# flo-stilz/Audio-Key-Estimation

Hardware: AMD Instinct MI355X
Metric: clips/s (15 s @ 22.05 kHz), HIP CQT + PitchClassNet forward (higher is better)
Workload: dtype f32 accumulation everywhere; pitch / semitone / layer-0 convolutions: f16 activations x f16 weights (per-channel power-of-two scaled) on MFMA, one product; last layer's pitch-class convolutions and heads: 3-term split-bf16 on MFMA (hi*hi + lo*hi + hi*lo); CQT filter bank: 3-term split-bf16 on MFMA

## Files before the change

### audio-key-estimation_amd/csrc/common.h

```cpp
#pragma once

#include <hip/hip_runtime.h>

#include <atomic>
#include <cstdarg>
#include <cstdint>
#include <cstdio>
#include <cstdlib>
#include <string>
#include <vector>

#include "../../include/ake_hip.h"

namespace ake {

void set_error(const char* fmt, ...);

#define AKE_HIP_CHECK(expr)                                                                  \
    do {                                                                                     \
        hipError_t _e = (expr);                                                              \
        if (_e != hipSuccess) {                                                              \
            ake::set_error("%s failed: %s (%s:%d)", #expr, hipGetErrorString(_e), __FILE__, __LINE__); \
            return AKE_ERR_HIP;                                                              \
        }                                                                                    \
// ... 16 lines not shown
bool prof_active();

struct DeviceOnce {
    std::atomic<uint64_t> done{0};
    static int dev() { int d = 0; (void)hipGetDevice(&d); return d & 63; }
    bool need() const { return !((done.load(std::memory_order_acquire) >> dev()) & 1); }
    void mark() { done.fetch_or(1ull << dev(), std::memory_order_release); }
};

template <typename... K>
int set_lds_limit(int bytes, K... kernels) {
    for (const void* f : {reinterpret_cast<const void*>(kernels)...})
        AKE_HIP_CHECK(hipFuncSetAttribute(f, hipFuncAttributeMaxDynamicSharedMemorySize, bytes));
    return AKE_OK;
}

template <typename... K>
int raise_lds_limit(DeviceOnce& once, int bytes, K... kernels) {
    if (!once.need()) return AKE_OK;
    const int rc = set_lds_limit(bytes, kernels...);
    if (!rc) once.mark();
    return rc;
}

template <typename... P, typename... A>
int launch_untimed(const char* name, void (*kernel)(P...), dim3 grid, dim3 block, size_t lds, hipStream_t s, const A&... args) {
    hipLaunchKernelGGL(kernel, grid, block, lds, s, static_cast<P>(args)...);
    const hipError_t e = hipGetLastError();
    if (e == hipSuccess) return AKE_OK;
    set_error("%s: launch failed: %s (grid %u x %u x %u, block %u x %u x %u, %zu B of dynamic LDS)", name, hipGetErrorString(e), grid.x, grid.y,
              grid.z, block.x, block.y, block.z, lds);
    return AKE_ERR_HIP;
}

template <typename... P, typename... A>
int launch(const char* name, void (*kernel)(P...), dim3 grid, dim3 block, size_t lds, hipStream_t s, const A&... args) {
    ProfScope ps(name, s);
    return launch_untimed(name, kernel, grid, block, lds, s, args...);
}

template <typename... P, typename... A>
int launch_flat(const char* name, void (*kernel)(P...), hipStream_t s, long long total, const A&... args) {
    return launch(name, kernel, dim3(static_cast<unsigned>((total + 255) / 256)), dim3(256), 0, s, args...);
}

__device__ __forceinline__ void lds_dma_16(const uint4* src, unsigned int lds_dst) {
    unsigned int keep;
    asm volatile("s_mov_b32 %0, m0\n\ts_mov_b32 m0, %2\n\ts_nop 0\n\tglobal_load_lds_dwordx4 %1, off\n\ts_mov_b32 m0, %0"
                 : "=&s"(keep) : "v"(src), "s"(lds_dst) : "memory");
}

int pcnet_local_window(const ake_pcnet* net);

inline size_t align_up(size_t v, size_t a) { return (v + a - 1) / a * a; }

struct Carver {
    char* base;
    size_t off;
    size_t cap;
    explicit Carver(void* b, size_t c) : base(static_cast<char*>(b)), off(0), cap(c) {}
    template <typename T>
    T* take(size_t n) {
        off = align_up(off, 256);
        T* p = base ? reinterpret_cast<T*>(base + off) : nullptr;
        off += n * sizeof(T);
        return p;
    }
};

}
```

### audio-key-estimation_amd/csrc/pcnet.hip

```cpp
#include <algorithm>
#include <cmath>
#include <cstdlib>
#include <cstring>
#include <map>
#include <string>
#include <vector>

#include "common.h"
#include "pcnet_kernels.h"
#include "pcnet_bwd_kernels.h"

using namespace ake_k;

namespace {

constexpr double kBnEps = 1e-5;
constexpr size_t kLdsBudget = 64 * 1024;
constexpr size_t kBfFragsPerConv = 14 * 2 * 64 + 64;

struct TensorSpec {
    std::string name;
    int64_t shape[4];
    int ndim;
};
// ... 2422 lines not shown
                    const PackedConv& px = train ? n->p2p[i][j].train : n->p2p[i][j].eval;
                    const int bn = train ? n->p2p[i][j].bn : -1;
                    P2pX3Opts ox;
                    ox.lrelu = !train;
                    if ((rc = run_p2p_f16x3(n, rk.x3[j > 0], px.bf_off, sdesc, in_aff, n->blob_dev + px.b_off, B, P, Ti, out.p, d.out_p,
                                            train ? b.stats + 2 * n->bns[bn].ch_off : nullptr, train ? 2 * n->bn_channels : 0, s, "conv_p2p_f16x3_kernel/p2p", ox)))
                        return rc;
                    if (train && (rc = finalize_bn(bn, static_cast<double>(B) * P * Ti, out.aff))) return rc;
                } else if ((rc = conv(n->p2p[i][j], 0, sdesc, in_aff, B, P, Ti, true, out.p, d.out_p, 0, out.aff, "conv_mfma_kernel/p2p")))
                    return rc;
                sdesc = Src{out.p, d.out_p, nullptr, 0, 0};
                in_aff = out.aff;
            }
            if (last_out == P2pOut::SemiFold) {
            } else if (last_out == P2pOut::Semi) {
                if ((rc = run_fold_max("fold_max_kernel", out.p, nullptr, d.out_p, P / 3, B, Ti, cat, ctot, d.prev_pc, s))) return rc;
            } else if (c.stay_sixth && train) {
                if ((rc = run_fold_max("fold_affine_kernel", out.p, out.aff, d.out_p, P, B, Ti, cat, ctot, d.prev_pc, s))) return rc;
                if ((rc = identity(b.aff_cat[i] + 3 * d.prev_pc, d.out_p))) return rc;
            } else if (c.stay_sixth) {
                if ((rc = fold_maps(i, out.p, d.out_p, P, B, Ti, cat, ctot, d.prev_pc))) return rc;
            } else if ((rc = semi(i, out.p, out.aff, B, P, Ti, cat, ctot, d.prev_pc, train ? b.aff_cat[i] + 3 * d.prev_pc : nullptr))) return rc;
            if (last) return AKE_OK;
            Slot psrc{cat, b.cat_slot(train, i).aff};
            int cin = ctot;
            Slot pdst;
            if (c.resblock && train) {
                if ((rc = res_stack_train(n->pc2pc[i], 1, Src{psrc.p, cin, nullptr, 0, 0}, psrc.aff, B, 12, Ti, b.pcst[i], b.aff_pcst[i],
                                          nullptr, 0, "conv_mfma_kernel/pc2pc")))
                    return rc;
                pdst = b.pc_last(i);
            } else if (c.resblock) {
                if ((rc = res_stack(n->pc2pc[i], 1, Src{psrc.p, cin, nullptr, 0, 0}, B, 12, Ti, b.pca[i], b.pcb[i], nullptr, 0, "conv_mfma_kernel/pc2pc"))) return rc;
                pdst = Slot{b.pca[i], nullptr};
            }
            for (int j = 0; j < c.conv_layers && !c.resblock; ++j) {
                pdst = b.pc_out(train, i, j);
                if ((rc = conv(n->pc2pc[i][j], 1, Src{psrc.p, cin, nullptr, 0, 0}, psrc.aff, B, 12, Ti, true, pdst.p, d.out_pc, 0, pdst.aff, "conv_mfma_kernel/pc2pc")))
                    return rc;
                psrc = pdst; cin = d.out_pc;
            }
            const LayerDims& dn = n->dims[i + 1];
            const int ctn = dn.prev_pc + dn.out_p;
            const int Tn = Ti / tp;
            float* catn = b.cat[i + 1] + (i + 1 == L - 1 ? static_cast<size_t>(c0) * ctn * 12 * Tn : 0);
            if ((rc = time_pool(pdst.p, pdst.aff, B, d.out_pc, 12, Ti, catn, ctn, 0))) return rc;
            if (train && (rc = identity(b.aff_cat[i + 1], d.out_pc))) return rc;
            if ((rc = time_pool(out.p, out.aff, B, d.out_p, P, Ti, b.ppool[i], d.out_p, 0))) return rc;
            pc_cur = catn; p_cur = b.ppool[i]; cp = d.out_p;
        }
        return AKE_OK;
    }

    int tail(int B, const int64_t* seq, float* key_out, float* tonic_out, float* genre_out) {
        const auto& c = n->cfg;
        const int L = c.num_layers, tp = c.time_pool_size;
        const int i = L - 1;
        const int Ti = b.Tl[i];
        const LayerDims& d = n->dims[i];
        int rc;
        Slot psrc = L == 1 ? Slot{b.fold0, nullptr} : b.cat_slot(train, i);
        int cin = L == 1 ? 1 : d.prev_pc + d.out_p;
        const int cout_default = L == 1 ? c.n_filters : d.out_pc;
        const int cout = cout_default;
        Slot pdst;
        const bool pc_bf = r.pc == PcStack::Bf16, pc_fused = r.pc == PcStack::Fused;
        const bool head_bf = r.heads != HeadForm::Generic;
        if (pc_fused) {
            if ((rc = run_pc2pc_fused(n, i, psrc.p, cin, B, Ti, b.pcf, head_bf ? b.feat_cl : nullptr, s))) return rc;
        } else if (pc_bf && (rc = run_nchw_to_cl16(psrc.p, cin, B, Ti, reinterpret_cast<unsigned short*>(b.pcb[i]), s))) return rc;
        const char* const pc_label = L == 1 ? "conv_mfma_kernel/pc2pc0" : "conv_mfma_kernel/pc2pc";
        if (c.resblock && train) {
            if ((rc = res_stack_train(n->pc2pc[i], 1, Src{psrc.p, cin, nullptr, 0, 0}, psrc.aff, B, 12, Ti, b.pcst[i], b.aff_pcst[i], nullptr, 0, pc_label)))
                return rc;
            pdst = b.pc_last(i);
        } else if (c.resblock) {
            if ((rc = res_stack(n->pc2pc[i], 1, Src{psrc.p, cin, nullptr, 0, 0}, B, 12, Ti, b.pca[i], b.pcb[i], nullptr, 0, pc_label))) return rc;
            pdst = Slot{b.pca[i], nullptr};
        }
        if (c.denseblock) {
            if ((rc = dense_stack(i, 1, psrc.p, n->final_ch, cin, B, 12, Ti, b.pca[i], pc_label))) return rc;
            pdst = Slot{psrc.p, nullptr};
        }
        for (int j = 0; j < c.conv_layers && !pc_fused && !c.resblock && !c.denseblock; ++j) {
            pdst = b.pc_out(train, i, j);
            if (pc_bf) {
                const bool last_conv = j == c.conv_layers - 1;
                const unsigned short* in = reinterpret_cast<const unsigned short*>(j == 0 ? b.pcb[i] : b.pc_out(false, i, j - 1).p);
                if ((rc = run_pc_bf16(n, n->pc2pc[i][j].eval, in, B, Ti, true, true, last_conv ? pdst.p : nullptr,
                                      last_conv ? nullptr : reinterpret_cast<unsigned short*>(pdst.p), s, "conv_pc_bf16_kernel/pc2pc")))
                    return rc;
                continue;
            }
            if (r.pc_x3_convs >> j & 1) {
                const PackedConv& pt = n->pc2pc[i][j].train;
                unsigned short* planes = reinterpret_cast<unsigned short*>(b.pcb[i]);
                if ((rc = run_nchw_to_cl16_f16x2(psrc.p, cin, B, Ti, psrc.aff, planes, s))) return rc;
                const int bn = n->pc2pc[i][j].bn;
                PcBf16Opts o;
                o.f16x3 = true; o.stats = b.stats + 2 * n->bns[bn].ch_off; o.stats_stride = 2 * n->bn_channels;
                if ((rc = run_pc_bf16(n, pt, planes, B, Ti, true, false, pdst.p, nullptr, s, "conv_pc_f16x3_kernel/pc2pc", o))) return rc;
                if ((rc = finalize_bn(bn, static_cast<double>(B) * 12 * Ti, pdst.aff))) return rc;
            } else if ((rc = conv(n->pc2pc[i][j], 1, Src{psrc.p, cin, nullptr, 0, 0}, psrc.aff, B, 12, Ti, true, pdst.p, cout, 0, pdst.aff, pc_label)))
                return rc;
            psrc = pdst; cin = cout;
        }
        Slot feat = pdst;
        if (pc_fused) feat = Slot{b.pcf, nullptr};
        else if (L > 1) {
            const int cout = c.denseblock ? n->final_ch : cout_default;
            if ((rc = time_pool(pdst.p, pdst.aff, B, cout, 12, Ti, b.pcf, cout, 0))) return rc;
            feat = Slot{b.pcf, nullptr};
        }
        const int Tf = b.Tf;
        const Head* const heads = n->heads;
        int Tm = Tf;
        bool head_planes_ready = false;
        int pooled_heads = 0;
        unsigned short* feat_cl = b.feat_cl;
        if (head_bf && !pc_fused && (rc = run_nchw_to_cl16(feat.p, n->final_ch, B, Tf, feat_cl, s))) return rc;
        const bool head1_bf = r.heads == HeadForm::Head1 || r.heads == HeadForm::Fused, genre_bf = r.genre_bf;
        const int T1 = r.T1, T2 = r.T2, TpB = r.TpB;
        const int nh_bf = genre_bf ? 3 : 2;
        float* const maps[3] = {b.map_k, b.map_t, b.map_g};
        float* const outs[3] = {key_out, tonic_out, genre_out};
        PoolArgs pool;
        pool.seq = reinterpret_cast<const long long*>(seq);
        pool.n_pool_layers = L - 1; pool.tp = tp; pool.shrink = (c.kernel_size - 1) * c.head_layers; pool.max_pool = c.max_pool; pool.clip0 = 0;
        if (r.heads == HeadForm::Fused) {
            const size_t hf_lds = r.hf_lds;
            HeadsFusedArgs ha;
            std::memset(&ha, 0, sizeof(ha));
            ha.xh = feat_cl; ha.xl = feat_cl + static_cast<long long>(B) * 12 * Tf * 16;
            for (int h = 0; h < nh_bf; ++h) {
                const PackedConv& p0 = heads[h].convs[0].eval;
                const PackedConv& p1 = heads[h].convs[1].eval;
                ha.bfragA[h] = n->bf_frags_dev + p0.bf_off; ha.biasA[h] = n->blob_dev + p0.b_off; ha.KHA[h] = p0.kh;
                ha.bfragB[h] = n->bf_frags_dev + p1.bf_off; ha.biasB[h] = n->blob_dev + p1.b_off; ha.KHB[h] = p1.kh;
                ha.dst[h] = maps[h];
                ha.pout[h] = outs[h];
            }
            if (genre_bf) { ha.hs[0] = 2; ha.hs[1] = 0; ha.hs[2] = 1; }
            else { ha.hs[0] = 0; ha.hs[1] = 1; ha.hs[2] = 1; }
            ha.batch = B; ha.T_in = Tf; ha.T1 = T1; ha.T2 = T2; ha.TpA = T1 + 8; ha.TpB = TpB; ha.JB = (T2 + 15) / 16;
            ha.fin_off = static_cast<int>(hf_lds / sizeof(float)) - 12 * T2;
            ha.pool = pool;
            static ake::DeviceOnce hf_attr;
            if ((rc = ake::raise_lds_limit(hf_attr, 150 * 1024, heads_fused_kernel<3>, heads_fused_kernel<4>))) return rc;
            rc = r.heads_mt == 3 ? ake::launch("heads_fused_kernel", heads_fused_kernel<3>, dim3(nh_bf * B), dim3(512), hf_lds, s, ha)
                                 : ake::launch("heads_fused_kernel", heads_fused_kernel<4>, dim3(nh_bf * B), dim3(512), hf_lds, s, ha);
            if (rc) return rc;
            pooled_heads = nh_bf;
            Tm = T2;
        } else if (head1_bf) {
            Head1BfArgs ha;
            std::memset(&ha, 0, sizeof(ha));
            for (int h = 0; h < nh_bf; ++h) {
                const PackedConv& p0 = heads[h].convs[0].eval;
                const PackedConv& p1 = heads[h].convs[1].eval;
                unsigned short* planes = reinterpret_cast<unsigned short*>(b.head_out(false, h, 0, false).p);
                if (h == 0) {
                    PcBf16Opts tonic;
                    tonic.pc2 = &heads[1].convs[0].eval; tonic.planes_out2 = reinterpret_cast<unsigned short*>(b.head_out(false, 1, 0, false).p);
                    if ((rc = run_pc_bf16(n, p0, feat_cl, B, Tf, false, true, nullptr, planes, s, "conv_pc_bf16_kernel/head", tonic))) return rc;
                }
                if (h == 2 && (rc = run_pc_bf16(n, p0, feat_cl, B, Tf, false, true, nullptr, planes, s, "conv_pc_bf16_kernel/genre_head")))
                    return rc;
                ha.xh[h] = planes; ha.xl[h] = planes + static_cast<long long>(B) * 12 * T1 * 32;
                ha.bfrag[h] = n->bf_frags_dev + p1.bf_off; ha.bias[h] = n->blob_dev + p1.b_off; ha.dst[h] = maps[h];
                ha.KH[h] = p1.kh; ha.circular[h] = p1.kh == 12 ? 1 : 0; ha.H_out[h] = ha.circular[h] ? 12 : 12 - p1.kh + 1;
            }
            ha.T_in = T1; ha.T_out = T2; ha.JB = (T2 + 15) / 16; ha.Tp = TpB;
            size_t lds = std::max(static_cast<size_t>(2) * 12 * ha.Tp * 4 * sizeof(uint4), static_cast<size_t>(8) * kHead1MT * 4 * 64 * sizeof(float));
            if (r.heads_pool) {
                ha.fin_off = static_cast<int>(lds / sizeof(float));
                lds += static_cast<size_t>(12) * T2 * sizeof(float);
                for (int h = 0; h < nh_bf; ++h) ha.pout[h] = outs[h];
                ha.pool = pool;
                pooled_heads = nh_bf;
            }
// ... 23 lines not shown
                    }
                    const int bn = cs.bn;
                    PcBf16Opts o;
                    o.f16x3 = true; o.stats = b.stats + 2 * n->bns[bn].ch_off; o.stats_stride = 2 * n->bn_channels;
                    if ((rc = run_pc_bf16(n, pt, b.feat_cl, B, Tcur, false, false, dst.p, nullptr, s,
                                          h == 2 ? "conv_pc_f16x3_kernel/genre_head" : "conv_pc_f16x3_kernel/head", o)))
                        return rc;
                    const int H_out = heads[h].kind == 2 ? 12 - pt.kh + 1 : 12;
                    if ((rc = finalize_bn(bn, static_cast<double>(B) * H_out * (Tcur - pt.kw + 1), dst.aff))) return rc;
                    continue;
                }
                if (train && lastj && j > 0 && pe.cout == 1 && pe.kw == 7 && !n->raw_w_off.empty()) {
                    const size_t lds = (static_cast<size_t>(hc) * 12 * Tcur + static_cast<size_t>(hc) * pe.kh * 7) * sizeof(float);
                    if (lds <= 150 * 1024 && Tcur - 6 >= 1) {
                        static ake::DeviceOnce hl_attr;
                        if ((rc = ake::raise_lds_limit(hl_attr, 150 * 1024, conv_head_last_kernel))) return rc;
                        if ((rc = ake::launch(h == 2 ? "conv_head_last_kernel/genre" : "conv_head_last_kernel", conv_head_last_kernel, dim3(B), dim3(384), lds, s,
                                              src.p, src.aff, n->blob_dev + n->raw_w_off[cs.w], n->blob_dev + n->raw_w_off[cs.b], dst.p, hc, pe.kh,
                                              heads[h].kind == 2 ? 0 : 1, Tcur, Tcur - 6)))
                            return rc;
                        continue;
                    }
                }
                if ((rc = conv(cs, heads[h].kind, Src{src.p, hc, nullptr, 0, 0}, src.aff, B, 12, Tcur, false, dst.p, pe.cout, 0, dst.aff,
                               h == 2 ? "conv_mfma_kernel/genre_head" : "conv_mfma_kernel/head")))
                    return rc;
            }
            Tm = Tf - c.head_layers * (c.kernel_size - 1);
        }
        if (c.local > 0) {
            AKE_REQUIRE(Tm >= c.local, AKE_ERR_INVALID, "pcnet --local: %d map frames are fewer than the pooling window %d", Tm, c.local);
            LocalPoolArgs la;
            std::memset(&la, 0, sizeof(la));
            la.maps[0] = b.map_k; la.maps[1] = b.map_t; la.maps[2] = c.genre ? b.map_g : nullptr;
            la.outs[0] = key_out; la.outs[1] = tonic_out; la.outs[2] = genre_out;
            la.Tm = Tm; la.Tq = Tm - c.local + 1; la.W = c.local; la.batch = B;
            return ake::launch("local_pool_kernel", local_pool_kernel, dim3(static_cast<unsigned>((static_cast<long long>(B) * 12 * Tm + 255) / 256), 3), dim3(256),
                               0, s, la);
        }
        PoolHeadArgs pa;
        std::memset(&pa, 0, sizeof(pa));
        pa.maps[0] = b.map_k; pa.maps[1] = b.map_t; pa.maps[2] = c.genre ? b.map_g : nullptr;
        for (int h = 0; h < pooled_heads; ++h) pa.maps[h] = nullptr;
        if (!pa.maps[0] && !pa.maps[1] && !pa.maps[2]) return AKE_OK;
        pa.outs[0] = key_out; pa.outs[1] = tonic_out; pa.outs[2] = genre_out;
        pa.rows[0] = 12; pa.rows[1] = 12; pa.rows[2] = 11;
        pa.Tm = Tm; pa.batch = B; pa.pool = pool;
        return ake::launch("head_pool_kernel", head_pool_kernel, dim3((B * 12 + 63) / 64, 3), dim3(64), 0, s, pa);
    }
};

int forward_impl(const ake_pcnet* n, bool train, const float* mel, int batch, int frames, const int64_t* seq_length, float* key_out,
                 float* tonic_out, float* genre_out, float* bn_stats_out, void* workspace, size_t ws_bytes, ake_stream_t stream,
                 bool mel_frames_major = false) {
    AKE_REQUIRE(n && mel && key_out && tonic_out, AKE_ERR_INVALID, "pcnet forward: null argument");
    AKE_REQUIRE(n->finalized, AKE_ERR_STATE, "pcnet: ake_pcnet_finalize has not been called");
    AKE_REQUIRE(train || !n->eval_frags_stale, AKE_ERR_STATE,
                "pcnet: the last weight load was ake_pcnet_load_for_training_f32 (training fragments only): call ake_pcnet_load_from_device_f32 before inference");
    AKE_REQUIRE(batch > 0 && frames > 0, AKE_ERR_INVALID, "pcnet: bad batch/frames");
    AKE_REQUIRE(!n->cfg.genre || genre_out, AKE_ERR_INVALID, "pcnet: genre head enabled but genre_out is null");
    const int chunk = train ? batch : std::min(batch, n->chunk_clips);
    Buffers b;
    int rc = plan_buffers(n, batch, chunk, frames, workspace, &b, train);
    if (rc) return rc;
    AKE_REQUIRE(workspace && ws_bytes >= b.bytes, AKE_ERR_WORKSPACE, "pcnet: workspace %zu < %zu bytes", ws_bytes, b.bytes);
    hipStream_t s = static_cast<hipStream_t>(stream);
    const Route route = build_route(n, train, batch, chunk, frames, mel, workspace, mel_frames_major);
    AKE_REQUIRE(!mel_frames_major || route.frames_major, AKE_ERR_UNSUPPORTED,
                "pcnet: this configuration does not take the frames-major input (ake_pcnet_accepts_frames_major)");
    if (train) AKE_HIP_CHECK(hipMemsetAsync(b.stats, 0, sizeof(double) * 2 * n->bn_channels * kStatSlots, s));
    Fwd f{n, b, s, train, route};
    if ((rc = f.entry(mel, batch))) return rc;
    for (int c0 = 0; c0 < batch && n->cfg.num_layers > 1; c0 += chunk) {
        const int B = std::min(chunk, batch - c0);
        if ((rc = f.pitch_chunk(mel + static_cast<size_t>(c0) * n->cfg.pitches * frames, c0, B))) return rc;
    }
    if ((rc = f.tail(batch, seq_length, key_out, tonic_out, genre_out))) return rc;
    if (train && bn_stats_out)
        AKE_HIP_CHECK(hipMemcpyAsync(bn_stats_out, b.bstats, sizeof(float) * 3 * n->bn_channels, hipMemcpyDeviceToDevice, s));
    return AKE_OK;
}

}

#include "pcnet_backward.h"

size_t ake_pcnet_grad_floats(const ake_pcnet* n) { return n ? n->grad_floats : 0; }

int64_t ake_pcnet_grad_offset(const ake_pcnet* n, const char* name) {
    if (!n || !name) return -1;
    auto it = n->spec_index.find(name);
    if (it == n->spec_index.end()) return -1;
    return static_cast<int64_t>(n->grad_off[it->second]);
}

int ake_pcnet_backward_f32(const ake_pcnet* n, const float* mel, int batch, int frames, const int64_t* seq_length, const float* key_out,
                           const float* d_key, const float* d_tonic, const float* d_genre, float* grads_out, int accumulate,
                           void* workspace, size_t ws_bytes, ake_stream_t stream) {
    AKE_REQUIRE(n && mel && key_out && d_key && d_tonic && grads_out, AKE_ERR_INVALID, "pcnet backward: null argument");
    AKE_REQUIRE(n->finalized, AKE_ERR_STATE, "pcnet: ake_pcnet_finalize has not been called");
    AKE_REQUIRE(!n->cfg.genre || d_genre, AKE_ERR_INVALID, "pcnet backward: genre head enabled but d_genre is null");
    AKE_REQUIRE(!(n->cfg.p2pc_conv && n->cfg.stay_sixth), AKE_ERR_UNSUPPORTED, "pcnet: training a --p2pc_conv --stay_sixth net is not built");
    Buffers b;
    int rc = plan_buffers(n, batch, batch, frames, workspace, &b, true);
    if (rc) return rc;
    AKE_REQUIRE(workspace && ws_bytes >= b.bytes, AKE_ERR_WORKSPACE, "pcnet backward: workspace %zu < %zu bytes", ws_bytes, b.bytes);
    hipStream_t s = static_cast<hipStream_t>(stream);
    AKE_HIP_CHECK(hipMemsetAsync(b.gslots, 0, sizeof(gfx_t) * n->grad_floats * kGradSlots, s));
    AKE_HIP_CHECK(hipMemsetAsync(b.stats2, 0, sizeof(double) * (static_cast<size_t>(3) * n->bn_channels * kBwdStatSlots + n->bns.size() * (kAmaxSlots / 2)), s));
    Bwd bw{n, b, s, b.gslots, batch};
    rc = bw.run(mel, seq_length, d_key, d_tonic, d_genre, key_out);
    if (rc) return rc;
    return launch_flat("grad_reduce_kernel", grad_reduce_kernel, s, n->grad_floats, b.gslots, grads_out, static_cast<long long>(n->grad_floats), accumulate ? 1 : 0);
}

int ake_pcnet_local_frames(const ake_pcnet* n, int frames, int* pooled_frames, int* map_frames) {
    AKE_REQUIRE(n && n->cfg.local > 0, AKE_ERR_STATE, "pcnet: the net was not created with local > 0");
    int t = frames;
    for (int i = 1; i < n->cfg.num_layers; ++i) t /= n->cfg.time_pool_size;
    t -= (n->cfg.kernel_size - 1) * n->cfg.head_layers;
    if (map_frames) *map_frames = t;
    if (pooled_frames) *pooled_frames = t - n->cfg.local + 1;
    return AKE_OK;
}

int ake_pcnet_forward_local_f32(const ake_pcnet* n, const float* mel, int batch, int frames, float* key_out, float* tonic_out, float* genre_out,
                                void* workspace, size_t ws_bytes, ake_stream_t stream) {
    AKE_REQUIRE(n && n->cfg.local > 0, AKE_ERR_STATE, "pcnet: the net was not created with local > 0");
    return forward_impl(n, false, mel, batch, frames, nullptr, key_out, tonic_out, genre_out, nullptr, workspace, ws_bytes, stream);
}
// ... 133 lines not shown
                ake::set_error("tap: '%s' is held as f16 words for the pitch conv that reads it; ake_debug_keep_taps(1) before the forward writes it as f32", name);
                return AKE_ERR_INVALID;
            }
            return set(b.psix[i], d.prev_pc, 36, Ti);
        }
        if (i >= 1 && nm == m + "cat") return set(b.cat[i], d.prev_pc + d.out_p, 12, Ti);
        if (i == L - 1 && i >= 1 && nm == m + "time_pool_pc") return set(b.pcf, d.out_pc, 12, b.Tf);
    }
    const int Tm = b.Tf - (c.kernel_size - 1) * c.head_layers;
    if (nm == "key_map") return set(b.map_k, 1, 12, Tm);
    if (nm == "tonic_map") return set(b.map_t, 1, 12, Tm);
    if (nm == "genre_map" && c.genre) return set(b.map_g, 1, 11, Tm);
    ake::set_error("tap: '%s' is not a materialised activation", name);
    return AKE_ERR_INVALID;
}

int ake_debug_keep_taps(int on) {
    const int old = g_keep_taps;
    g_keep_taps = on != 0;
    return old;
}

int ake_pcnet_tap_info(const ake_pcnet* n, const char* name, int batch, int frames, int64_t shape[4]) {
    float* p = nullptr;
    return tap_lookup(n, name, batch, frames, nullptr, &p, shape);
}

int ake_pcnet_tap_copy(const ake_pcnet* n, const char* name, int batch, int frames, const void* workspace, float* out_dev,
                       ake_stream_t stream) {
    AKE_REQUIRE(workspace && out_dev, AKE_ERR_INVALID, "tap_copy: null argument");
    float* p = nullptr;
    int64_t shape[4];
    int cl = 0;
    long long clip_stride = 0;
    int rc = tap_lookup(n, name, batch, frames, workspace, &p, shape, &cl, &clip_stride);
    if (rc) return rc;
    if (clip_stride) {
        const size_t row = sizeof(float) * shape[1] * shape[2] * shape[3];
        AKE_HIP_CHECK(hipMemcpy2DAsync(out_dev, row, p, sizeof(float) * clip_stride, row, shape[0], hipMemcpyDeviceToDevice, static_cast<hipStream_t>(stream)));
        return AKE_OK;
    }
    if (cl) {
        const long long total = shape[0] * shape[1] * shape[2] * shape[3];
        const unsigned short* h = reinterpret_cast<const unsigned short*>(p);
        return ake::launch_untimed("cl_to_nchw_kernel", cl_to_nchw_kernel, dim3(static_cast<unsigned>((total + 255) / 256)), dim3(256), 0,
                                   static_cast<hipStream_t>(stream), h, cl == 2 ? nullptr : h + total, out_dev, shape[1], shape[2], shape[3], total);
    }
    AKE_HIP_CHECK(hipMemcpyAsync(out_dev, p, sizeof(float) * shape[0] * shape[1] * shape[2] * shape[3], hipMemcpyDeviceToDevice,
                                 static_cast<hipStream_t>(stream)));
    return AKE_OK;
}

}
```

### audio-key-estimation_amd/csrc/pcnet_kernels.h

```cpp
#pragma once

#include <hip/hip_runtime.h>

#include "common.h"

namespace ake_k {

constexpr int TW = 4;
constexpr float kSlope = 0.01f;

struct ConvArgs {
    const float* src0;
    const float* src1;
    long long src0_clip_stride, src1_clip_stride;
    int c0, c1, h1;
    int H;
    int T_in;
    int T_out;
    int H_out;
    int py;
    int pad_l;
    int time_circ;
    const float* w;
    const float* bias;
// ... 163 lines not shown
    for (int k = threadIdx.x; k < 2 * C; k += blockDim.x)
        if (sh[k] != 0) atomicAdd(reinterpret_cast<unsigned long long*>(stats + static_cast<size_t>(blockIdx.x & (kStatSlots - 1)) * stats_stride + k),
                                  static_cast<unsigned long long>(sh[k]));
}

template <bool TRAIN>
__global__ void up_sixth_kernel(const float* __restrict__ src, long long src_clip_stride, const float* __restrict__ in_aff,
                                const float* __restrict__ w, const float* __restrict__ bias, float* __restrict__ dst,
                                double* __restrict__ stats, int stats_stride, int C, int T, long long total) {
    __shared__ long long sh[TRAIN ? 2 * kBlockStatCh : 1];
    if constexpr (TRAIN) block_stats_begin(sh, C);
    const long long i = static_cast<long long>(blockIdx.x) * blockDim.x + threadIdx.x;
    if (i < total) {
        const int t = static_cast<int>(i % T);
        long long q = i / T;
        const int row = static_cast<int>(q % 36);
        q /= 36;
        const int co = static_cast<int>(q % C);
        const long long clip = q / C;
        const int p = row / 3, j = row - 3 * p;
        const float* s = src + clip * src_clip_stride + static_cast<long long>(p) * T + t;
        float acc = bias[co];
        for (int ci = 0; ci < C; ++ci) {
            const float x = s[static_cast<long long>(ci) * 12 * T];
            acc = fmaf(TRAIN ? affine_act(x, in_aff, ci) : x, w[(ci * C + co) * 3 + j], acc);
        }
        if constexpr (TRAIN) {
            dst[i] = acc;
            block_stats_add(sh, co, acc);
        } else dst[i] = acc > 0.f ? acc : acc * kSlope;
    }
    if constexpr (TRAIN) block_stats_end(sh, C, stats, stats_stride);
}

__global__ void time_pool_kernel(const float* __restrict__ src, const float* __restrict__ aff, float* __restrict__ dst, int C, int H, int T, int tp,
                                 int dst_ctot, int dst_coff, long long total) {
    const long long i = static_cast<long long>(blockIdx.x) * blockDim.x + threadIdx.x;
    if (i >= total) return;
    const int To = T / tp;
    const int t = static_cast<int>(i % To);
    long long q = i / To;
    const int y = static_cast<int>(q % H);
    q /= H;
    const int c = static_cast<int>(q % C);
    const long long clip = q / C;
    const float* s = src + ((clip * C + c) * H + y) * T + static_cast<long long>(t) * tp;
    float m = affine_act(s[0], aff, c);
    for (int j = 1; j < tp; ++j) m = fmaxf(m, affine_act(s[j], aff, c));
    dst[((clip * dst_ctot + dst_coff + c) * H + y) * To + t] = m;
}

struct PoolArgs {
    const long long* seq;
    int n_pool_layers;
    int tp;
    int shrink;
    int max_pool;
    int clip0;
};

struct PoolHeadArgs {
    const float* maps[3];
    float* outs[3];
    int rows[3];
    int Tm;
    int batch;
    PoolArgs pool;
};

__device__ __forceinline__ float pool_row(const PoolArgs& p, const float* m, int clip, int Tm, int head) {
    int L = Tm;
    bool use_max = p.max_pool != 0;
    if (p.seq) {
        long long l = p.seq[clip];
        for (int k = 0; k < p.n_pool_layers; ++k) l = l / p.tp;
        L = static_cast<int>(l) - p.shrink;
        if (L > Tm) L = Tm;
        if (L < 0) L = Tm + L > 0 ? Tm + L : 0;
        use_max = use_max && (p.clip0 + clip == 0);
    }
    float v;
    if (use_max) {
        v = -INFINITY;
        for (int t = 0; t < L; ++t) v = fmaxf(v, m[t]);
    } else {
        float sum = 0.f;
        for (int t = 0; t < L; ++t) sum += m[t];
        v = sum / static_cast<float>(L > 0 ? L : 0);
    }
    if (head == 0) v = 1.f / (1.f + expf(-v));
    return v;
}

__global__ void head_pool_kernel(PoolHeadArgs a) {
    const int i = blockIdx.x * blockDim.x + threadIdx.x;
    const int which = blockIdx.y;
    if (a.maps[which] == nullptr) return;
    const int rows = a.rows[which];
    if (i >= a.batch * rows) return;
    a.outs[which][i] = pool_row(a.pool, a.maps[which] + static_cast<long long>(i) * a.Tm, i / rows, a.Tm, which);
}


__global__ void concat_repeat_kernel(const float* __restrict__ src0, int c0, const float* __restrict__ src1, int c1, int h1, float* __restrict__ dst,
                                     int ctot, int H, int T, long long total, const float* __restrict__ aff1 = nullptr) {
    const long long i = static_cast<long long>(blockIdx.x) * blockDim.x + threadIdx.x;
    if (i >= total) return;
    const int t = static_cast<int>(i % T);
    long long r = i / T;
    const int y = static_cast<int>(r % H); r /= H;
    const int c = static_cast<int>(r % (c0 + c1));
    const long long clip = r / (c0 + c1);
    float v = c < c0 ? src0[((clip * c0 + c) * H + y) * T + t] : src1[((clip * c1 + (c - c0)) * h1 + y % h1) * T + t];
    if (aff1 && c >= c0) { const float x = fmaf(v, aff1[3 * (c - c0)], aff1[3 * (c - c0) + 1]); v = x > 0.f ? x : x * aff1[3 * (c - c0) + 2]; }
    dst[((clip * ctot + c) * H + y) * T + t] = v;
}

__global__ void dense_affine_kernel(const float* __restrict__ params, const int* __restrict__ idx, float* __restrict__ out, int n) {
    const int i = blockIdx.x * blockDim.x + threadIdx.x;
    if (i >= n) return;
    const int* o = idx + 5 * i;
    const double sc = static_cast<double>(params[o[0]]) / sqrt(static_cast<double>(params[o[3]]) + 1e-5);
    out[3 * i] = static_cast<float>(sc);
    out[3 * i + 1] = static_cast<float>(static_cast<double>(params[o[1]]) - static_cast<double>(params[o[2]]) * sc);
    out[3 * i + 2] = __int_as_float(o[4]);
}

// ... 1155 lines not shown
            int y = m0 / a.T_out, t = m0 - y * a.T_out;
#pragma unroll
            for (int i = 0; i < 4; ++i) {
                if (m0 + i < Mtot && co < a.cout) {
                    float v = F16X3 ? fmaf(fmaf(accl[F16X3 ? mt : 0][F16X3 ? nt : 0][i], kP2pLoInv, acc[mt][nt][i]), iscale, bias) : acc[mt][nt][i] + bias;
                    if (F16X3) sstat.add(v);
                    if (a.lrelu) v = v > 0.f ? v : v * kSlope;
                    if (OUT_CL) {
                        const long long idx = ((static_cast<long long>(clip) * H_out + y) * a.T_out + t) * a.cl_stride + co;
                        const unsigned int hb = bf16_bits(v);
                        oh[idx] = static_cast<unsigned short>(hb);
                        ol[idx] = static_cast<unsigned short>(bf16_bits(v - __uint_as_float(hb << 16)));
                    } else {
                        float* const d = a.dst + clip * a.dst_clip_stride + (static_cast<long long>(co) * H_out + y) * a.T_out + t;
                        *d = (F16X3 && a.accumulate) ? *d + v : v;
                    }
                }
                if (++t == a.T_out) { t = 0; ++y; }
            }
        }
        if (F16X3 && a.stats) {
            long long st1, st2;
            sstat.fixed(st1, st2);
            st1 += shfl_xor_ll(st1, 16); st2 += shfl_xor_ll(st2, 16);
            st1 += shfl_xor_ll(st1, 32); st2 += shfl_xor_ll(st2, 32);
            if (q == 0 && co < a.cout) {
                double* st = a.stats + static_cast<size_t>((blockIdx.x + 7 * blockIdx.z + wave) & (kStatSlots - 1)) * a.stats_stride;
                fx_add_int(st + 2 * co, st1);
                fx_add_int(st + 2 * co + 1, st2);
            }
        }
    }
}

struct Pc2pcFusedArgs {
    const float* src;
    long long src_clip_stride;
    int cin, n_conv;
    const uint4* bfrag[4];
    const float* bias[4];
    float* pooled;
    unsigned short* fh;
    unsigned short* fl;
    int T, Tp;
};

__global__ __launch_bounds__(1024) void pc2pc_fused_kernel(Pc2pcFusedArgs a) {
    extern __shared__ __attribute__((aligned(16))) uint4 lds4[];
    const int clip = blockIdx.x;
    const int lane = threadIdx.x & 63;
    const int wave = __builtin_amdgcn_readfirstlane(threadIdx.x >> 6);
    const int r16 = lane & 15, q = lane >> 4;
    const int T = a.T, Tp = a.Tp;
    constexpr int MT = 4;
    const int n16 = 12 * Tp * 2;
    uint4* const map0 = lds4;
    uint4* const map1 = lds4 + 2 * n16;
    uint4* const wring = lds4 + 4 * n16;
    constexpr int kRow = 4 * 2 * 64;
    for (int i = threadIdx.x; i < 4 * n16; i += 1024) lds4[i] = make_uint4(0, 0, 0, 0);
    const int wsrc0 = (((threadIdx.x >> 7) * 4) * 2 + ((threadIdx.x >> 6) & 1)) * 64 + (threadIdx.x & 63);
    auto wsrc = [&](int p, int dq) { return wsrc0 + (16 * dq * 2 + p * 2) * 64; };
    if (threadIdx.x < kRow) wring[threadIdx.x] = a.bfrag[0][wsrc(0, 0)];
    __syncthreads();
    {
        const float* src = a.src + clip * a.src_clip_stride;
        for (int i = threadIdx.x; i < 12 * T * 2; i += 1024) {
            const int half = i & 1, pos = i >> 1;
            const int y = pos / T, t = pos - y * T;
            unsigned int hi[4] = {0, 0, 0, 0}, lo[4] = {0, 0, 0, 0};
#pragma unroll
            for (int k = 0; k < 8; ++k) {
                const int c = half * 8 + k;
                const float v = c < a.cin ? src[(static_cast<long long>(c) * 12 + y) * T + t] : 0.f;
                const unsigned int hb = bf16_bits(v);
                hi[k >> 1] |= hb << (16 * (k & 1));
                lo[k >> 1] |= bf16_bits(v - __uint_as_float(hb << 16)) << (16 * (k & 1));
            }
            const int idx = ((y * Tp + t + 3) << 1) + half;
            map0[idx] = make_uint4(hi[0], hi[1], hi[2], hi[3]);
            map0[n16 + idx] = make_uint4(lo[0], lo[1], lo[2], lo[3]);
        }
    }
    __syncthreads();
    const int n_tt = (T + 15) >> 4;
    const bool active = wave < 3 * n_tt;
    const int tt = wave / 3, y0 = 4 * (wave - 3 * tt);
    const int t0 = 16 * tt;
    const int dxq = q >> 1, half = q & 1;
    const int lane_off = ((t0 + r16 + dxq) << 1) + half;
    const int lane_off3 = ((t0 + r16 + 6) << 1) + half;
    auto frag_off = [&](int s, int p) {
        int row = y0 + s + (p == 3 ? dxq : 0);
        row -= row >= 12 ? 12 : 0;
        return ((row * Tp) << 1) + (p == 3 ? lane_off3 : lane_off + 4 * p);
    };
    const int Tf = T / 2;
    float* const pooled_c = a.pooled + static_cast<long long>(clip) * 16 * 12 * Tf;
    unsigned short* const fh_c = a.fh ? a.fh + static_cast<long long>(clip) * 12 * Tf * 16 : nullptr;
    unsigned short* const fl_c = a.fh ? a.fl + static_cast<long long>(clip) * 12 * Tf * 16 : nullptr;
    for (int j = 0; j < a.n_conv; ++j) {
        const uint4* const pH = (j & 1) ? map1 : map0;
        const uint4* const pL = pH + n16;
        unsigned short* const oH = reinterpret_cast<unsigned short*>((j & 1) ? map0 : map1);
        unsigned short* const oL = oH + n16 * 8;
        const bool last = j == a.n_conv - 1;
        const uint4* const bfrag_j = j == 0 ? a.bfrag[0] : (j == 1 ? a.bfrag[1] : (j == 2 ? a.bfrag[2] : a.bfrag[3]));
        const float* const bias_j = j == 0 ? a.bias[0] : (j == 1 ? a.bias[1] : (j == 2 ? a.bias[2] : a.bias[3]));
        const uint4* const bfrag_n = j == 0 ? a.bfrag[1] : (j == 1 ? a.bfrag[2] : a.bfrag[3]);
        {
            f32x4c acc[MT];
#pragma unroll
            for (int mt = 0; mt < MT; ++mt) acc[mt] = f32x4c{0.f, 0.f, 0.f, 0.f};
            bf16x8c fh[4], fl[4];
            int c = 0;
            auto run_p = [&](auto pair_c, const int p) __attribute__((always_inline)) {
                constexpr bool PAIR = decltype(pair_c)::value;
                if (active) {
#pragma unroll
                    for (int s = 0; s < 4; ++s) {
                        const int off = frag_off(s, PAIR ? 3 : p);
                        fh[s] = __builtin_bit_cast(bf16x8c, pH[off]);
                        fl[s] = __builtin_bit_cast(bf16x8c, pL[off]);
                    }
                }
#pragma unroll 1
                for (int dq = 0; dq < 3; ++dq, ++c) {
                    uint4 wpre = make_uint4(0, 0, 0, 0);
                    const bool fetch = threadIdx.x < kRow && (c + 1 < 12 || j + 1 < a.n_conv);
                    if (fetch) wpre = c + 1 < 12 ? bfrag_j[dq < 2 ? wsrc(p, dq + 1) : wsrc(p + 1, 0)] : bfrag_n[wsrc(0, 0)];
                    const uint4* const wr = wring + (c & 1) * kRow + lane;
                    if (active) {
#pragma unroll
                        for (int i = 0; i < 4; i += PAIR ? 2 : 1) {
                            const bf16x8c bh = __builtin_bit_cast(bf16x8c, wr[(i * 2 + 0) * 64]), bl = __builtin_bit_cast(bf16x8c, wr[(i * 2 + 1) * 64]);
#pragma unroll
                            for (int mt = 0; mt < MT; ++mt) acc[mt] = __builtin_amdgcn_mfma_f32_16x16x32_bf16(fh[(mt + i) & 3], bh, acc[mt], 0, 0, 0);
#pragma unroll
                            for (int mt = 0; mt < MT; ++mt) acc[mt] = __builtin_amdgcn_mfma_f32_16x16x32_bf16(fl[(mt + i) & 3], bh, acc[mt], 0, 0, 0);
#pragma unroll
                            for (int mt = 0; mt < MT; ++mt) acc[mt] = __builtin_amdgcn_mfma_f32_16x16x32_bf16(fh[(mt + i) & 3], bl, acc[mt], 0, 0, 0);
#pragma unroll
                            for (int u = 0; u < (PAIR ? 2 : 1); ++u) {
                                const int s_new = 4 * dq + i + 4 + u;
                                if (s_new < 12 + MT - (PAIR ? 2 : 1)) {
                                    const int off = frag_off(s_new, PAIR ? 3 : p);
                                    fh[i + u] = __builtin_bit_cast(bf16x8c, pH[off]);
                                    fl[i + u] = __builtin_bit_cast(bf16x8c, pL[off]);
                                }
                            }
                        }
                    }
                    if (fetch) wring[((c + 1) & 1) * kRow + threadIdx.x] = wpre;
                    if (c + 1 < 12) __syncthreads();
                }
            };
#pragma unroll 1
            for (int p = 0; p < 3; ++p) run_p(std::false_type{}, p);
            run_p(std::true_type{}, 3);
            if (active) {
            const int co = r16;
            const float bias = bias_j[co];
            const int tq0 = t0 + 4 * q;
            if (tq0 < T) {
#pragma unroll
            for (int mt = 0; mt < MT; ++mt) {
                    const int y = y0 + mt;
                    float v[4];
#pragma unroll
                    for (int i = 0; i < 4; ++i) {
                        const float x = acc[mt][i] + bias;
                        v[i] = x > 0.f ? x : x * kSlope;
                    }
                    if (!last) {
#pragma unroll
                        for (int i = 0; i < 4; ++i) {
                            const int e = ((((y * Tp + tq0 + i + 3) << 1) + (co >> 3)) << 3) + (co & 7);
                            const unsigned int hb = bf16_bits(v[i]);
                            oH[e] = static_cast<unsigned short>(hb);
                            oL[e] = static_cast<unsigned short>(bf16_bits(v[i] - __uint_as_float(hb << 16)));
                        }
                    } else {
#pragma unroll
                        for (int i = 0; i < 4; i += 2) {
                            const float pv = fmaxf(v[i], v[i + 1]);
                            const int tq = (tq0 + i) >> 1;
                            pooled_c[(co * 12 + y) * Tf + tq] = pv;
                            if (a.fh) {
                                const int e = (y * Tf + tq) * 16 + co;
                                const unsigned int hb = bf16_bits(pv);
                                fh_c[e] = static_cast<unsigned short>(hb);
                                fl_c[e] = static_cast<unsigned short>(bf16_bits(pv - __uint_as_float(hb << 16)));
                            }
                        }
                    }
            }
            }
            }
        }
        __syncthreads();
    }
}

struct Head1BfArgs {
    const unsigned short* xh[3];
    const unsigned short* xl[3];
    const uint4* bfrag[3];
    const float* bias[3];
    float* dst[3];
    int KH[3], H_out[3], circular[3];
    int T_in, T_out, Tp, JB;
    float* pout[3];
    PoolArgs pool;
    int fin_off;
};

constexpr int kHead1MT = 4;
constexpr int kHead1JB = 5;
__host__ __device__ constexpr int head1_ksteps(int KH) { return KH == 12 ? 12 * 7 : KH * 22; }
constexpr int kHead1PF = 3;

__device__ __forceinline__ void head1_prefetch(const uint4* __restrict__ bg, int nks, int wave, uint4 (&nbh)[kHead1PF], uint4 (&nbl)[kHead1PF]) {
#pragma unroll
    for (int i = 0; i < kHead1PF; ++i) {
        const int kn = wave + 8 * i < nks ? wave + 8 * i : wave;
        nbh[i] = bg[(2 * kn + 0) * 64]; nbl[i] = bg[(2 * kn + 1) * 64];
    }
}

__device__ __forceinline__ void head1_multiply_store(const uint4* __restrict__ bg, int nks, uint4 (&nbh)[kHead1PF], uint4 (&nbl)[kHead1PF], uint4* lds4,
                                                     int Tp, int HO, int circ, int JB, int T_out, int clip, const float* bias_p, float* dst,
                                                     bool keep, int fin_off) {
    constexpr int PF = kHead1PF;
    const int lane = threadIdx.x & 63;
    const int wave = __builtin_amdgcn_readfirstlane(threadIdx.x >> 6);
    const int r16 = lane & 15, q = lane >> 4;
    const uint4* const pH = lds4;
    const uint4* const pL = lds4 + 12 * Tp * 4;
    float* const red = reinterpret_cast<float*>(lds4);
    if (circ) {
        f32x4c acc[kHead1JB];
#pragma unroll
        for (int mt = 0; mt < kHead1JB; ++mt) acc[mt] = f32x4c{0.f, 0.f, 0.f, 0.f};
        for (int ks = wave; ks < nks; ks += 8) {
            const int r = ks / 7, dx = ks - r * 7;
            const bf16x8c bh = __builtin_bit_cast(bf16x8c, nbh[0]);
            const bf16x8c bl = __builtin_bit_cast(bf16x8c, nbl[0]);
#pragma unroll
            for (int i = 0; i + 1 < PF; ++i) { nbh[i] = nbh[i + 1]; nbl[i] = nbl[i + 1]; }
            {
                const int kn = ks + 8 * PF < nks ? ks + 8 * PF : ks;
                nbh[PF - 1] = bg[(2 * kn + 0) * 64]; nbl[PF - 1] = bg[(2 * kn + 1) * 64];
// ... 1287 lines not shown
```

### audio-key-estimation_amd/csrc/pipeline.hip

```cpp
#include "common.h"

namespace {

__global__ void fill_i64_kernel(long long* dst, long long v, int n) {
    const int i = blockIdx.x * blockDim.x + threadIdx.x;
    if (i < n) dst[i] = v;
}

__global__ void frames_i64_kernel(long long* dst, const long long* __restrict__ n_clip, int hop, long long t_max, int n) {
    const int i = blockIdx.x * blockDim.x + threadIdx.x;
    if (i < n) {
        const long long nc = n_clip[i];
        const long long t = nc < 0 ? 0 : 1 + nc / hop;
        dst[i] = t < t_max ? t : t_max;
    }
}

struct PipeCarve {
    float* mel;
    long long* seq;
    void* cqt_ws;
    size_t cqt_bytes;
    void* net_ws;
    size_t net_bytes;
    size_t total;
};

int carve(const ake_cqt_plan* plan, const ake_pcnet* net, int batch, int64_t n, int n_bins, void* ws, PipeCarve* pc) {
    const int64_t T = ake_cqt_num_frames(plan, n);
    AKE_REQUIRE(T > 0, AKE_ERR_INVALID, "pipeline: bad n_samples");
    ake::Carver c(ws, 0);
    pc->mel = c.take<float>(static_cast<size_t>(batch) * n_bins * T);
    pc->seq = c.take<long long>(batch);
    pc->cqt_bytes = ake_cqt_workspace_bytes(plan, batch, n);
    pc->cqt_ws = c.take<char>(pc->cqt_bytes);
    pc->net_bytes = ake_pcnet_workspace_bytes(net, batch, static_cast<int>(T));
    pc->net_ws = c.take<char>(pc->net_bytes);
    pc->total = ake::align_up(c.off, 256);
    return AKE_OK;
}

}

extern "C" {

size_t ake_pipeline_workspace_bytes(const ake_cqt_plan* plan, const ake_pcnet* net, int batch, int64_t n_samples) {
    if (!plan || !net || batch <= 0 || n_samples <= 0) return 0;
    PipeCarve pc;
    if (carve(plan, net, batch, n_samples, ake_cqt_plan_n_bins(plan), nullptr, &pc) != AKE_OK) return 0;
    return pc.total;
}

static int pipeline_impl(const ake_cqt_plan* plan, const ake_pcnet* net, const float* audio_dev, int batch, int64_t n_samples,
                         int64_t audio_stride, const int64_t* n_clip_dev, int hop, float* key_out_dev, float* tonic_out_dev,
                         float* genre_out_dev, void* workspace, size_t workspace_bytes, ake_stream_t stream, const int16_t* pcm16_dev = nullptr);

int ake_pipeline_forward_f32(const ake_cqt_plan* plan, const ake_pcnet* net, const float* audio_dev, int batch,
                             int64_t n_samples, int64_t audio_stride, float* key_out_dev, float* tonic_out_dev,
                             float* genre_out_dev, void* workspace, size_t workspace_bytes, ake_stream_t stream) {
    return pipeline_impl(plan, net, audio_dev, batch, n_samples, audio_stride, nullptr, 0, key_out_dev, tonic_out_dev, genre_out_dev, workspace,
                         workspace_bytes, stream);
}

int ake_pipeline_forward_ragged_f32(const ake_cqt_plan* plan, const ake_pcnet* net, const float* audio_dev, int batch,
                                    int64_t n_max, int64_t audio_stride, const int64_t* n_samples_dev, float* key_out_dev,
                                    float* tonic_out_dev, float* genre_out_dev, void* workspace, size_t workspace_bytes,
                                    ake_stream_t stream) {
    AKE_REQUIRE(n_samples_dev, AKE_ERR_INVALID, "ake_pipeline_forward_ragged_f32: null n_samples_dev");
    AKE_REQUIRE(plan && n_max > 0, AKE_ERR_INVALID, "ake_pipeline_forward_ragged_f32: bad argument");
    return pipeline_impl(plan, net, audio_dev, batch, n_max, audio_stride, n_samples_dev, ake_cqt_plan_hop(plan), key_out_dev, tonic_out_dev,
                         genre_out_dev, workspace, workspace_bytes, stream);
}

int ake_pipeline_forward_pcm16_f32(const ake_cqt_plan* plan, const ake_pcnet* net, const int16_t* audio_dev, int batch, int64_t n_max,
                                   int64_t audio_stride, const int64_t* n_samples_dev, float* key_out_dev, float* tonic_out_dev,
                                   float* genre_out_dev, void* workspace, size_t workspace_bytes, ake_stream_t stream) {
    AKE_REQUIRE(plan && n_max > 0, AKE_ERR_INVALID, "ake_pipeline_forward_pcm16_f32: bad argument");
    return pipeline_impl(plan, net, nullptr, batch, n_max, audio_stride, n_samples_dev, ake_cqt_plan_hop(plan), key_out_dev, tonic_out_dev,
                         genre_out_dev, workspace, workspace_bytes, stream, audio_dev);
}

static int pipeline_impl(const ake_cqt_plan* plan, const ake_pcnet* net, const float* audio_dev, int batch, int64_t n_samples,
                         int64_t audio_stride, const int64_t* n_clip_dev, int hop, float* key_out_dev, float* tonic_out_dev,
                         float* genre_out_dev, void* workspace, size_t workspace_bytes, ake_stream_t stream, const int16_t* pcm16_dev) {
    AKE_REQUIRE(plan && net && (audio_dev || pcm16_dev), AKE_ERR_INVALID, "ake_pipeline_forward_f32: null argument");
    const int n_bins = ake_cqt_plan_n_bins(plan);
    AKE_REQUIRE(n_bins == ake_pcnet_pitches(net), AKE_ERR_INVALID, "pipeline: CQT has %d bins but the net expects %d pitches",
                n_bins, ake_pcnet_pitches(net));
    PipeCarve pc;
    int rc = carve(plan, net, batch, n_samples, n_bins, workspace, &pc);
    if (rc) return rc;
    AKE_REQUIRE(workspace && workspace_bytes >= pc.total, AKE_ERR_WORKSPACE, "pipeline: workspace %zu < %zu bytes", workspace_bytes, pc.total);
    const int64_t T = ake_cqt_num_frames(plan, n_samples);
    hipStream_t s = static_cast<hipStream_t>(stream);
    const bool fm = !n_clip_dev && ake_cqt_frames_major_supported(plan) && ake_pcnet_accepts_frames_major(net, batch, static_cast<int>(T));
    rc = pcm16_dev  ? ake_cqt_logmag_pcm16_f32(plan, pcm16_dev, batch, n_samples, audio_stride, n_clip_dev, nullptr, pc.mel, T, fm ? 1 : 0, pc.cqt_ws, pc.cqt_bytes, stream)
         : n_clip_dev ? ake_cqt_logmag_ragged_f32(plan, audio_dev, batch, n_samples, audio_stride, n_clip_dev, pc.mel, T, pc.cqt_ws, pc.cqt_bytes, stream)
         : fm       ? ake_cqt_logmag_frames_major_f32(plan, audio_dev, batch, n_samples, audio_stride, pc.mel, pc.cqt_ws, pc.cqt_bytes, stream)
                    : ake_cqt_logmag_f32(plan, audio_dev, batch, n_samples, audio_stride, pc.mel, T, pc.cqt_ws, pc.cqt_bytes, stream);
    if (rc) return rc;
    if (n_clip_dev)
        rc = ake::launch_untimed("frames_i64_kernel", frames_i64_kernel, dim3((batch + 255) / 256), dim3(256), 0, s, pc.seq,
                                 reinterpret_cast<const long long*>(n_clip_dev), hop, T, batch);
    else
        rc = ake::launch_untimed("fill_i64_kernel", fill_i64_kernel, dim3((batch + 255) / 256), dim3(256), 0, s, pc.seq, T, batch);
    if (rc) return rc;
    if (fm)
        return ake_pcnet_forward_frames_major_f32(net, pc.mel, batch, static_cast<int>(T), reinterpret_cast<const int64_t*>(pc.seq), key_out_dev,
                                                  tonic_out_dev, genre_out_dev, pc.net_ws, pc.net_bytes, stream);
    return ake_pcnet_forward_f32(net, pc.mel, batch, static_cast<int>(T), reinterpret_cast<const int64_t*>(pc.seq), key_out_dev,
                                 tonic_out_dev, genre_out_dev, pc.net_ws, pc.net_bytes, stream);
}

}
```

Before: 465,100.

## Pass uniform sequence length as scalar and split last time tile across extra waves

For the uniform-length pipeline path, the fill kernel that wrote a per-clip sequence-length array is dropped, and the frame count is passed as a scalar through PoolArgs into the pooling code. That removes one small kernel launch and a global read per clip. Separately, the fused pc2pc conv kernel now uses idle waves when there are five time tiles: waves 12+ take the last tile with three rows each (MT=3) instead of leaving it to fewer waves, which improves wave utilisation but adds code paths and register pressure.

```diff
diff --git a/audio-key-estimation_amd/csrc/common.h b/audio-key-estimation_amd/csrc/common.h
--- a/audio-key-estimation_amd/csrc/common.h
+++ b/audio-key-estimation_amd/csrc/common.h
@@ -92,6 +92,9 @@
 
 int pcnet_local_window(const ake_pcnet* net);
 
+int pcnet_forward_uniform(const ake_pcnet* net, const float* mel, int batch, int frames, long long seq_all, bool frames_major, float* key_out,
+                          float* tonic_out, float* genre_out, void* workspace, size_t ws_bytes, ake_stream_t stream);
+
 inline size_t align_up(size_t v, size_t a) { return (v + a - 1) / a * a; }
 
 struct Carver {
diff --git a/audio-key-estimation_amd/csrc/pcnet.hip b/audio-key-estimation_amd/csrc/pcnet.hip
--- a/audio-key-estimation_amd/csrc/pcnet.hip
+++ b/audio-key-estimation_amd/csrc/pcnet.hip
@@ -2498,7 +2498,7 @@
         return AKE_OK;
     }
 
-    int tail(int B, const int64_t* seq, float* key_out, float* tonic_out, float* genre_out) {
+    int tail(int B, const int64_t* seq, long long seq_all, float* key_out, float* tonic_out, float* genre_out) {
         const auto& c = n->cfg;
         const int L = c.num_layers, tp = c.time_pool_size;
         const int i = L - 1;
@@ -2571,7 +2571,7 @@
         float* const maps[3] = {b.map_k, b.map_t, b.map_g};
         float* const outs[3] = {key_out, tonic_out, genre_out};
         PoolArgs pool;
-        pool.seq = reinterpret_cast<const long long*>(seq);
+        pool.seq = reinterpret_cast<const long long*>(seq); pool.seq_all = seq ? -1 : seq_all;
         pool.n_pool_layers = L - 1; pool.tp = tp; pool.shrink = (c.kernel_size - 1) * c.head_layers; pool.max_pool = c.max_pool; pool.clip0 = 0;
         if (r.heads == HeadForm::Fused) {
             const size_t hf_lds = r.hf_lds;
@@ -2701,7 +2701,7 @@
 
 int forward_impl(const ake_pcnet* n, bool train, const float* mel, int batch, int frames, const int64_t* seq_length, float* key_out,
                  float* tonic_out, float* genre_out, float* bn_stats_out, void* workspace, size_t ws_bytes, ake_stream_t stream,
-                 bool mel_frames_major = false) {
+                 bool mel_frames_major = false, long long seq_all = -1) {
     AKE_REQUIRE(n && mel && key_out && tonic_out, AKE_ERR_INVALID, "pcnet forward: null argument");
     AKE_REQUIRE(n->finalized, AKE_ERR_STATE, "pcnet: ake_pcnet_finalize has not been called");
     AKE_REQUIRE(train || !n->eval_frags_stale, AKE_ERR_STATE,
@@ -2724,7 +2724,7 @@
         const int B = std::min(chunk, batch - c0);
         if ((rc = f.pitch_chunk(mel + static_cast<size_t>(c0) * n->cfg.pitches * frames, c0, B))) return rc;
     }
-    if ((rc = f.tail(batch, seq_length, key_out, tonic_out, genre_out))) return rc;
+    if ((rc = f.tail(batch, seq_length, seq_all, key_out, tonic_out, genre_out))) return rc;
     if (train && bn_stats_out)
         AKE_HIP_CHECK(hipMemcpyAsync(bn_stats_out, b.bstats, sizeof(float) * 3 * n->bn_channels, hipMemcpyDeviceToDevice, s));
     return AKE_OK;
@@ -2964,3 +2964,11 @@
 }
 
 }
+
+int ake::pcnet_forward_uniform(const ake_pcnet* n, const float* mel, int batch, int frames, long long seq_all, bool frames_major, float* key_out,
+                               float* tonic_out, float* genre_out, void* workspace, size_t ws_bytes, ake_stream_t stream) {
+    AKE_REQUIRE(!n || n->cfg.local == 0 || frames_major, AKE_ERR_STATE, "pcnet: a --local net returns per-frame outputs: call ake_pcnet_forward_local_f32");
+    AKE_REQUIRE(!n || n->cfg.local == 0, AKE_ERR_UNSUPPORTED, "pcnet: a --local net does not take the frames-major input");
+    AKE_REQUIRE(seq_all >= 0, AKE_ERR_INVALID, "pcnet: bad uniform seq_length %lld", seq_all);
+    return forward_impl(n, false, mel, batch, frames, nullptr, key_out, tonic_out, genre_out, nullptr, workspace, ws_bytes, stream, frames_major, seq_all);
+}
diff --git a/audio-key-estimation_amd/csrc/pcnet_kernels.h b/audio-key-estimation_amd/csrc/pcnet_kernels.h
--- a/audio-key-estimation_amd/csrc/pcnet_kernels.h
+++ b/audio-key-estimation_amd/csrc/pcnet_kernels.h
@@ -239,6 +239,7 @@
 
 struct PoolArgs {
     const long long* seq;
+    long long seq_all;
     int n_pool_layers;
     int tp;
     int shrink;
@@ -258,8 +259,8 @@
 __device__ __forceinline__ float pool_row(const PoolArgs& p, const float* m, int clip, int Tm, int head) {
     int L = Tm;
     bool use_max = p.max_pool != 0;
-    if (p.seq) {
-        long long l = p.seq[clip];
+    if (p.seq || p.seq_all >= 0) {
+        long long l = p.seq ? p.seq[clip] : p.seq_all;
         for (int k = 0; k < p.n_pool_layers; ++k) l = l / p.tp;
         L = static_cast<int>(l) - p.shrink;
         if (L > Tm) L = Tm;
@@ -1521,7 +1522,6 @@
     const int wave = __builtin_amdgcn_readfirstlane(threadIdx.x >> 6);
     const int r16 = lane & 15, q = lane >> 4;
     const int T = a.T, Tp = a.Tp;
-    constexpr int MT = 4;
     const int n16 = 12 * Tp * 2;
     uint4* const map0 = lds4;
     uint4* const map1 = lds4 + 2 * n16;
@@ -1553,8 +1553,9 @@
     }
     __syncthreads();
     const int n_tt = (T + 15) >> 4;
-    const bool active = wave < 3 * n_tt;
-    const int tt = wave / 3, y0 = 4 * (wave - 3 * tt);
+    const bool active = wave < 3 * n_tt || n_tt == 5;
+    const bool rows3 = n_tt == 5 && wave >= 12;
+    const int tt = rows3 ? 4 : wave / 3, y0 = rows3 ? 3 * (wave - 12) : 4 * (wave - 3 * tt);
     const int t0 = 16 * tt;
     const int dxq = q >> 1, half = q & 1;
     const int lane_off = ((t0 + r16 + dxq) << 1) + half;
@@ -1577,7 +1578,8 @@
         const uint4* const bfrag_j = j == 0 ? a.bfrag[0] : (j == 1 ? a.bfrag[1] : (j == 2 ? a.bfrag[2] : a.bfrag[3]));
         const float* const bias_j = j == 0 ? a.bias[0] : (j == 1 ? a.bias[1] : (j == 2 ? a.bias[2] : a.bias[3]));
         const uint4* const bfrag_n = j == 0 ? a.bfrag[1] : (j == 1 ? a.bfrag[2] : a.bfrag[3]);
-        {
+        auto conv = [&](auto mt_c) __attribute__((always_inline)) {
+            constexpr int MT = decltype(mt_c)::value;
             f32x4c acc[MT];
 #pragma unroll
             for (int mt = 0; mt < MT; ++mt) acc[mt] = f32x4c{0.f, 0.f, 0.f, 0.f};
@@ -1666,7 +1668,9 @@
             }
             }
             }
-        }
+        };
+        if (rows3) conv(std::integral_constant<int, 3>{});
+        else conv(std::integral_constant<int, 4>{});
         __syncthreads();
     }
 }
diff --git a/audio-key-estimation_amd/csrc/pipeline.hip b/audio-key-estimation_amd/csrc/pipeline.hip
--- a/audio-key-estimation_amd/csrc/pipeline.hip
+++ b/audio-key-estimation_amd/csrc/pipeline.hip
@@ -1,11 +1,6 @@
 #include "common.h"
 
 namespace {
-
-__global__ void fill_i64_kernel(long long* dst, long long v, int n) {
-    const int i = blockIdx.x * blockDim.x + threadIdx.x;
-    if (i < n) dst[i] = v;
-}
 
 __global__ void frames_i64_kernel(long long* dst, const long long* __restrict__ n_clip, int hop, long long t_max, int n) {
     const int i = blockIdx.x * blockDim.x + threadIdx.x;
@@ -99,15 +94,12 @@
          : fm       ? ake_cqt_logmag_frames_major_f32(plan, audio_dev, batch, n_samples, audio_stride, pc.mel, pc.cqt_ws, pc.cqt_bytes, stream)
                     : ake_cqt_logmag_f32(plan, audio_dev, batch, n_samples, audio_stride, pc.mel, T, pc.cqt_ws, pc.cqt_bytes, stream);
     if (rc) return rc;
-    if (n_clip_dev)
-        rc = ake::launch_untimed("frames_i64_kernel", frames_i64_kernel, dim3((batch + 255) / 256), dim3(256), 0, s, pc.seq,
-                                 reinterpret_cast<const long long*>(n_clip_dev), hop, T, batch);
-    else
-        rc = ake::launch_untimed("fill_i64_kernel", fill_i64_kernel, dim3((batch + 255) / 256), dim3(256), 0, s, pc.seq, T, batch);
+    if (!n_clip_dev)
+        return ake::pcnet_forward_uniform(net, pc.mel, batch, static_cast<int>(T), T, fm, key_out_dev, tonic_out_dev, genre_out_dev, pc.net_ws,
+                                          pc.net_bytes, stream);
+    rc = ake::launch_untimed("frames_i64_kernel", frames_i64_kernel, dim3((batch + 255) / 256), dim3(256), 0, s, pc.seq,
+                             reinterpret_cast<const long long*>(n_clip_dev), hop, T, batch);
     if (rc) return rc;
-    if (fm)
-        return ake_pcnet_forward_frames_major_f32(net, pc.mel, batch, static_cast<int>(T), reinterpret_cast<const int64_t*>(pc.seq), key_out_dev,
-                                                  tonic_out_dev, genre_out_dev, pc.net_ws, pc.net_bytes, stream);
     return ake_pcnet_forward_f32(net, pc.mel, batch, static_cast<int>(T), reinterpret_cast<const int64_t*>(pc.seq), key_out_dev,
                                  tonic_out_dev, genre_out_dev, pc.net_ws, pc.net_bytes, stream);
 }
```

Result: faster. 471,000, median of 6 (+1.3%).
